# Jack-Tattershall/mujoco-manip

Measured on AMD Instinct MI355X. Metric: env steps/sec (whole node) at 4096 parallel envs; 1/2/4/8 MI355X scaling, higher is better.
Workload: dtype f32

## Files before the change

mujoco_manip_amd/_build.py:

```python
from __future__ import annotations

import os
import subprocess
from concurrent.futures import ThreadPoolExecutor

PKG = os.path.dirname(os.path.abspath(__file__))
CSRC = os.path.join(PKG, "csrc")
LIB = os.path.join(PKG, "libmmx.so")
LIB_PROF = os.path.join(PKG, "libmmx_prof.so")
SOURCES = ["mmx_kernels.hip", "mmx_step_l192.hip", "mmx_render.hip", "mmx_render_lit.hip", "mmx_png.hip",
           "mmx_snapshot.hip", "mmx_mppi.hip", "mmx_policy.hip", "mmx_api.cpp"]
ARCH = os.environ.get("MMX_OFFLOAD_ARCH", "gfx950")
DEVICE_MATH = ["-Xarch_device", "-freciprocal-math", "-Xarch_device", "-fapprox-func",
               "-Xarch_device", "-ffinite-math-only", "-Xarch_device", "-fno-signed-zeros"]
DEVICE_SCHED = ["-mllvm", "-amdgpu-sched-strategy=" + os.environ.get("MMX_SCHED", "iterative-ilp")]
if os.environ.get("MMX_SCHED") == "default":
    DEVICE_SCHED = []
DEVICE_NOSLP = ["-Xarch_device", "-fno-slp-vectorize"]
FLAGS = DEVICE_MATH + DEVICE_SCHED + DEVICE_NOSLP + os.environ.get("MMX_EXTRA_FLAGS", "").split()
SOURCE_FLAGS = {"mmx_kernels.hip": ["-Xarch_device", "-fassociative-math"],
                "mmx_step_l192.hip": ["-Xarch_device", "-fassociative-math"],
                "mmx_mppi.hip": ["-Xarch_device", "-fno-finite-math-only"]}


STEP_SOURCES = ["mmx_kernels.hip", "mmx_step_l192.hip"]
HIPCC_JOBS = 16
TEST_VARIANTS = {
    "libmmx_col4.so": ["MMX_COL_LIST=4", "MMX_CAND_CAP=4"],
    "libmmx_nolist.so": ["MMX_CAND_CAP=1"],
    "libmmx_hdelay.so": ["MMX_HELPER_DELAY=1", "MMX_PROBE=14"],
    "libmmx_edelay.so": ["MMX_HELPER_DELAY=2", "MMX_PROBE=14"],
    "libmmx_synth.so": ["MMX_BUDGET_SYNTH=1"],
}


def lib_path(profile: bool = False) -> str:
    return LIB_PROF if profile else LIB


def test_variant(name: str) -> str:
    path = os.path.join(PKG, name)
    if not os.path.exists(path):
        raise RuntimeError("test build missing: run __graft_entry__.build()")
    return path


def _stale(lib: str) -> bool:
    if not os.path.exists(lib):
        return True
    t = os.path.getmtime(lib)
    inc = os.path.join(PKG, "..", "include")
    deps = [os.path.join(CSRC, f) for f in os.listdir(CSRC) if f.endswith((".hip", ".cpp", ".h", ".inc"))]
    deps += [os.path.join(inc, f) for f in os.listdir(inc) if f.endswith(".h")]
    return any(os.path.getmtime(d) > t for d in deps)


def _hipcc(src: str, obj: str, defines: list[str] | tuple = (), profile: bool = False, verbose: bool = False) -> str:
    cmd = [os.environ.get("HIPCC", "/opt/rocm/bin/hipcc")] + (["-xhip"] if src.endswith(".cpp") else [])
    cmd += FLAGS + SOURCE_FLAGS.get(src, []) + [f"-D{d}" for d in defines] + (["-DMMX_PHASE_CLOCK=1"] if profile else [])
    cmd += [f"--offload-arch={ARCH}", "-O3", "-std=c++17", "-fPIC", "-c", os.path.join(CSRC, src), "-o", obj]
    if verbose:
        print(" ".join(cmd), flush=True)
    subprocess.check_call(cmd)
    return obj


def _link(out: str, objs: list[str]) -> str:
    subprocess.check_call([os.environ.get("HIPCC", "/opt/rocm/bin/hipcc"), f"--offload-arch={ARCH}", "-shared", "-fPIC", "-o", out] + objs)
    return out


def _obj(src: str, tag: str = "") -> str:
    return os.path.join(CSRC, os.path.splitext(src)[0] + tag + ".o")


def build(force: bool = False, verbose: bool = False, profile: bool | None = False) -> str:
    variants = [False, True] if profile is None else [profile]
    variants = [v for v in variants if force or _stale(lib_path(v))]
    tests = [n for n in TEST_VARIANTS if profile is None and (force or _stale(os.path.join(PKG, n)))]
    if variants or tests:
        pdef = [f"MMX_PROBE={int(os.environ.get('MMX_PROBE', '1'))}"]
        jobs = [(src, v) for v in variants for src in SOURCES]
        tjobs = [(n, src) for n in tests for src in STEP_SOURCES]
        with ThreadPoolExecutor(max_workers=min(HIPCC_JOBS, len(jobs) + len(tjobs))) as ex:
            tobjs = [ex.submit(_hipcc, src, _obj(src, "_" + os.path.splitext(n)[0]), TEST_VARIANTS[n], False, verbose)
                     for n, src in tjobs]
            objs = list(ex.map(lambda j: _hipcc(j[0], _obj(j[0], "_prof" if j[1] else ""), pdef if j[1] else [], j[1], verbose), jobs))
            tobjs = [f.result() for f in tobjs]
        for v in variants:
            _link(lib_path(v), [o for o, (_, vv) in zip(objs, jobs) if vv == v])
        for n in tests:
            kobjs = [o for o, (nn, _) in zip(tobjs, tjobs) if nn == n]
            _link(os.path.join(PKG, n), kobjs + [_obj(src) for src in SOURCES if src not in STEP_SOURCES])
    return lib_path(bool(profile))


if __name__ == "__main__":
    print(build(force=True, verbose=True, profile=None))


def build_variant(out: str, defines: list[str], profile: bool = True) -> str:
    tag = os.path.splitext(os.path.basename(out))[0]
    where = os.path.dirname(os.path.abspath(out))
    os.makedirs(where, exist_ok=True)
    with ThreadPoolExecutor(max_workers=len(SOURCES)) as ex:
        objs = list(ex.map(lambda src: _hipcc(src, os.path.join(where, f"{tag}_{os.path.splitext(src)[0]}.o"), defines, profile), SOURCES))
    return _link(out, objs)
```

mujoco_manip_amd/csrc/mmx_geom.h:

```cpp
#ifndef MMX_GEOM_H
#define MMX_GEOM_H
#include "mmx_device.h"
#include "mmx_state.h"
#include "mmx_clock.h"

enum { GT_PLANE = 0, GT_CYL = 5, GT_BOX = 6, GT_MESH = 7 };

struct Geom {
  V3 x;
  M3 R;
  int type, g;
};

DEV V3 support(const Geom& G, V3 dir) {
  V3 dl = mulT(G.R, dir), sl;
  const int g = G.g;
  if (G.type == GT_BOX) {
    sl = V3{dl.x >= 0.f ? MMX_geom_size[3 * g] : -MMX_geom_size[3 * g],
            dl.y >= 0.f ? MMX_geom_size[3 * g + 1] : -MMX_geom_size[3 * g + 1],
            dl.z >= 0.f ? MMX_geom_size[3 * g + 2] : -MMX_geom_size[3 * g + 2]};
  } else if (G.type == GT_CYL) {
    const float r = MMX_geom_size[3 * g], hh = MMX_geom_size[3 * g + 1];
    const float n = sqrtf(dl.x * dl.x + dl.y * dl.y);
    sl = n > 1e-12f ? V3{r * dl.x / n, r * dl.y / n, 0.f} : V3{r, 0.f, 0.f};
    sl.z = dl.z >= 0.f ? hh : -hh;
  } else {
    const int m = MMX_geom_mesh[g];
    const int a = MMX_mesh_vertadr[m], nvert = MMX_mesh_vertnum[m];
    float best = -3.0e38f;
    int bi = a;
    for (int v = a; v < a + nvert; v++) {
      const float s = MMX_mesh_vert[3 * v] * dl.x + MMX_mesh_vert[3 * v + 1] * dl.y + MMX_mesh_vert[3 * v + 2] * dl.z;
      if (s > best) {
        best = s;
        bi = v;
      }
    }
    sl = V3{MMX_mesh_vert[3 * bi], MMX_mesh_vert[3 * bi + 1], MMX_mesh_vert[3 * bi + 2]};
  }
  return G.x + mul(G.R, sl);
}

DEV bool obb_overlap(const Geom& A, const Geom& B, V3 ha, V3 hb) {
  const V3 d = B.x - A.x;
  float Rm[3][3], aR[3][3];
#pragma unroll
  for (int i = 0; i < 3; i++)
#pragma unroll
    for (int j = 0; j < 3; j++) {
      Rm[i][j] = dot(col(A.R, i), col(B.R, j));
      aR[i][j] = fabsf(Rm[i][j]);
    }
  const float hA[3] = {ha.x, ha.y, ha.z}, hB[3] = {hb.x, hb.y, hb.z};
  bool sep = false;
#pragma unroll
  for (int i = 0; i < 3; i++) {
    const float t = dot(d, col(A.R, i));
    sep |= fabsf(t) > hA[i] + hB[0] * aR[i][0] + hB[1] * aR[i][1] + hB[2] * aR[i][2];
  }
#pragma unroll
  for (int j = 0; j < 3; j++) {
    const float u = dot(d, col(B.R, j));
    sep |= fabsf(u) > hB[j] + hA[0] * aR[0][j] + hA[1] * aR[1][j] + hA[2] * aR[2][j];
  }
  (void)Rm;
  return !sep;
}

template <class Sink>
DEV void plane_box(Sink& cs, const Geom& P, const Geom& B, V3 hb) {
  const V3 nz = col(P.R, 2);
  const float h[3] = {hb.x, hb.y, hb.z};
  float cd[8];
  V3 cp[8];
  int cnt = 0;
#pragma unroll
  for (int k = 0; k < 8; k++) {
    cd[k] = 0.f;
    cp[k] = V3{0.f, 0.f, 0.f};
  }
#pragma unroll
  for (int k = 0; k < 8; k++) {
    const V3 l = V3{(k & 1) ? h[0] : -h[0], (k & 2) ? h[1] : -h[1], (k & 4) ? h[2] : -h[2]};
    const V3 w = B.x + mul(B.R, l);
    const float d = dot(w - P.x, nz);
    if (d <= 0.f) {
      const V3 pw = w - nz * (0.5f * d);
// ... 359 lines not shown
  wave_argmax(best, bi);
  const int wl = bi & 63;
  const V3 p = V3{__int_as_float(__builtin_amdgcn_readlane(__float_as_int(bx), wl)),
                  __int_as_float(__builtin_amdgcn_readlane(__float_as_int(by), wl)),
                  __int_as_float(__builtin_amdgcn_readlane(__float_as_int(bz), wl))};
  return G.x + mul(G.R, p);
}

struct SVx {
  V3 w, a, b;
};
struct GPair {
  const Geom& A;
  const Geom& B;
};
DEV SVx mk_sv(const GPair& P, V3 dir) {
  SVx s;
  s.a = support_wave(P.A, dir);
  s.b = support_wave(P.B, -dir);
  s.w = s.a - s.b;
  return s;
}
DEV bool gjk_line(const SVx& s0, const SVx& s1, int& n, V3& dir) {
  const V3 ab = s1.w - s0.w, ao = -s0.w;
  if (dot(ab, ao) > 0.f) {
    dir = cross(cross(ab, ao), ab);
    n = 2;
    return norm(dir) < 1e-12f * (1.f + dot(ab, ab));
  }
  n = 1;
  dir = ao;
  return false;
}
DEV bool gjk_tri(const SVx& s0, SVx& s1, SVx& s2, int& n, V3& dir) {
  const V3 ab = s1.w - s0.w, ac = s2.w - s0.w, ao = -s0.w;
  const V3 abc = cross(ab, ac);
  if (dot(cross(abc, ac), ao) > 0.f) {
    if (dot(ac, ao) > 0.f) {
      s1 = s2;
      n = 2;
      dir = cross(cross(ac, ao), ac);
      return false;
    }
    n = 2;
    return gjk_line(s0, s1, n, dir);
  }
  if (dot(cross(ab, abc), ao) > 0.f) {
    n = 2;
    return gjk_line(s0, s1, n, dir);
  }
  const float dd = dot(abc, ao);
  n = 3;
  if (fabsf(dd) < 1e-12f * (1.f + dot(abc, abc))) return true;
  if (dd > 0.f) dir = abc;
  else {
    const SVx t = s1;
    s1 = s2;
    s2 = t;
    dir = -abc;
  }
  return false;
}
DEV bool gjk_face_out(const SVx& s0, const SVx& b, const SVx& c, const SVx& o) {
  V3 nn = cross(b.w - s0.w, c.w - s0.w);
  if (dot(nn, o.w - s0.w) > 0.f) nn = -nn;
  return dot(nn, -s0.w) > 0.f;
}
DEV bool gjk_tet(const SVx& s0, SVx& s1, SVx& s2, SVx& s3, int& n, V3& dir) {
  n = 3;
  if (gjk_face_out(s0, s1, s2, s3)) return gjk_tri(s0, s1, s2, n, dir);
  if (gjk_face_out(s0, s2, s3, s1)) {
    s1 = s2;
    s2 = s3;
    return gjk_tri(s0, s1, s2, n, dir);
  }
  if (gjk_face_out(s0, s3, s1, s2)) {
    s2 = s1;
    s1 = s3;
    return gjk_tri(s0, s1, s2, n, dir);
  }
  n = 4;
  return true;
}
DEV bool gjk(const GPair& GP, SVx& s0, SVx& s1, SVx& s2, SVx& s3, int& n) {
  V3 dir = GP.A.x - GP.B.x;
  if (norm(dir) < 1e-9f) dir = V3{1.f, 0.f, 0.f};
  s0 = mk_sv(GP, dir);
  n = 1;
  dir = -s0.w;
  for (int it = 0; it < 48; it++) {
    if (norm(dir) < 1e-12f) return true;
    const SVx P = mk_sv(GP, dir);
    if (dot(P.w, dir) < 0.f) return false;
    s3 = s2;
    s2 = s1;
    s1 = s0;
    s0 = P;
    n++;
    const bool hit = n == 2 ? gjk_line(s0, s1, n, dir)
                            : (n == 3 ? gjk_tri(s0, s1, s2, n, dir) : gjk_tet(s0, s1, s2, s3, n, dir));
    if (hit) return true;
  }
  return norm(dir) < 1e-12f;
}

#define EPA_MAXV 38
#define EPA_MAXF 72
struct EFace {
  int vv;
  V3 n;
  float d;
  DEV int v(int k) const { return (vv >> (8 * k)) & 255; }
};
static_assert(EPA_MAXV < 256, "EPA vertex indices are packed in bytes");
DEV bool epa_face(const SVx* V, EFace& f, int a, int b, int c) {
  f.vv = a | (b << 8) | (c << 16);
  const V3 n = cross(V[b].w - V[a].w, V[c].w - V[a].w);
  const float ln = norm(n);
  if (ln < 1e-20f) return false;
  f.n = n * (1.f / ln);
  f.d = dot(f.n, V[a].w);
  return true;
}
DEV void epa_sync() {
  __builtin_amdgcn_fence(__ATOMIC_RELEASE, "wavefront");
  __builtin_amdgcn_wave_barrier();
  __builtin_amdgcn_fence(__ATOMIC_ACQUIRE, "wavefront");
}
DEV int epa_lane() { return (int)(threadIdx.x & 63); }
DEV int epa_prefix(unsigned long long m) {
  return __builtin_amdgcn_mbcnt_hi((unsigned)(m >> 32), __builtin_amdgcn_mbcnt_lo((unsigned)m, 0u));
}
DEV bool epa(const GPair& GP, SVx* V, int nv, V3& nrm, float& depth, V3& pa, V3& pb, EFace* F, int* edges) {
  int nf = 0;
  if (nv == 1) {
    for (int k = 0; k < 6 && nv < 2; k++) {
      const float sg = (k & 1) ? -1.f : 1.f;
      V[nv] = mk_sv(GP, V3{k < 2 ? sg : 0.f, (k >> 1) == 1 ? sg : 0.f, k >= 4 ? sg : 0.f});
      if (norm(V[nv].w - V[0].w) > 1e-7f) nv++;
    }
  }
  if (nv == 2) {
    const V3 ab = V[1].w - V[0].w;
    const V3 ax = fabsf(ab.x) <= fabsf(ab.y) && fabsf(ab.x) <= fabsf(ab.z)
                      ? V3{1.f, 0.f, 0.f}
                      : (fabsf(ab.y) <= fabsf(ab.z) ? V3{0.f, 1.f, 0.f} : V3{0.f, 0.f, 1.f});
    const V3 t = normalize(cross(ab, ax));
    V[2] = mk_sv(GP, t);
    if (norm(cross(V[2].w - V[0].w, ab)) < 1e-10f) V[2] = mk_sv(GP, -t);
    nv = 3;
  }
  if (nv == 3) {
    const V3 n = normalize(cross(V[1].w - V[0].w, V[2].w - V[0].w));
    V[3] = mk_sv(GP, n);
    if (fabsf(dot(V[3].w - V[0].w, n)) < 1e-9f) V[3] = mk_sv(GP, -n);
    nv = 4;
  }
  const int T[4][3] = {{0, 1, 2}, {0, 3, 1}, {0, 2, 3}, {1, 3, 2}};
  const V3 cen = (V[0].w + V[1].w + V[2].w + V[3].w) * 0.25f;
  for (int k = 0; k < 4; k++) {
    if (!epa_face(V, F[nf], T[k][0], T[k][1], T[k][2])) continue;
    if (dot(F[nf].n, V[T[k][0]].w - cen) < 0.f) epa_face(V, F[nf], T[k][0], T[k][2], T[k][1]);
    nf++;
  }
  static_assert(EPA_MAXF <= 128, "two faces per lane");
  const int ln = epa_lane();
  int best = -1;
  for (;;) {
    epa_sync();
    float bd = -3e38f;
    int bi = 0x7fffffff;
    if (ln < nf && F[ln].d < 3e38f) {
      bd = -F[ln].d;
      bi = ln;
    }
// ... 3 lines not shown
    }
    wave_argmax(bd, bi);
    best = bi < nf ? bi : -1;
    if (best < 0) return false;
    const V3 fn = F[best].n;
    const float fd = F[best].d;
    const SVx P = mk_sv(GP, fn);
    const float dist = dot(P.w, fn);
    if (dist - fd < 1e-6f * (1.f + fabsf(dist)) || nv >= EPA_MAXV) break;
    EFace f0, f1;
    bool vis0 = false, vis1 = false;
    if (ln < nf) {
      f0 = F[ln];
      vis0 = dot(f0.n, P.w - V[f0.v(0)].w) > 1e-9f;
    }
    if (ln + 64 < nf) {
      f1 = F[ln + 64];
      vis1 = dot(f1.n, P.w - V[f1.v(0)].w) > 1e-9f;
    }
    const unsigned long long mv0 = __ballot(vis0), mv1 = __ballot(vis1);
    const unsigned long long mk0 = __ballot(ln < nf && !vis0), mk1 = __ballot(ln + 64 < nf && !vis1);
    int ne = 0;
    for (int half = 0; half < 2; half++) {
      unsigned long long m = half ? mv1 : mv0;
      while (m) {
        const int k = 64 * half + __builtin_ctzll(m);
        m &= m - 1ull;
        const EFace f = F[k];
        for (int e = 0; e < 3; e++) {
          const int a = f.v(e), b = f.v((e + 1) % 3);
          int found = -1;
          for (int q0 = 0; q0 < ne && found < 0; q0 += 64) {
            const int q = q0 + ln;
            const unsigned long long hit = __ballot(q < ne && edges[q] == (b | (a << 8)));
            if (hit) found = q0 + __builtin_ctzll(hit);
          }
          epa_sync();
          if (found >= 0) {
            if (ln == 0) edges[found] = edges[ne - 1];
            ne--;
          } else if (ne < EPA_MAXF * 3) {
            if (ln == 0) edges[ne] = a | (b << 8);
            ne++;
          }
          epa_sync();
        }
      }
    }
    epa_sync();
    const int nk0 = __popcll(mk0);
    if (ln < nf && !vis0) F[epa_prefix(mk0)] = f0;
    if (ln + 64 < nf && !vis1) F[nk0 + epa_prefix(mk1)] = f1;
    nf = nk0 + __popcll(mk1);
    const int pi = nv++;
    if (ln == 0) V[pi] = P;
    epa_sync();
    for (int q0 = 0; q0 < ne && nf < EPA_MAXF; q0 += 64) {
      const int q = q0 + ln;
      EFace g;
      const bool ok = q < ne && epa_face(V, g, edges[q] & 255, edges[q] >> 8, pi);
      const unsigned long long mo = __ballot(ok);
      const int pos = nf + epa_prefix(mo);
      if (ok && pos < EPA_MAXF) F[pos] = g;
      nf = min(EPA_MAXF, nf + __popcll(mo));
    }
  }
  epa_sync();
  if (best < 0) return false;
  const EFace& f = F[best];
  const V3 p = f.n * f.d;
  const V3 ra = V[f.v(0)].w - p, rb = V[f.v(1)].w - p, rc = V[f.v(2)].w - p;
  const float den = dot(cross(V[f.v(1)].w - V[f.v(0)].w, V[f.v(2)].w - V[f.v(0)].w), f.n);
  const float lu = den > 1e-15f ? dot(cross(rb, rc), f.n) / den : 1.f;
  const float lv = den > 1e-15f ? dot(cross(rc, ra), f.n) / den : 0.f;
  const float lw = 1.f - lu - lv;
  pa = V[f.v(0)].a * lu + V[f.v(1)].a * lv + V[f.v(2)].a * lw;
  pb = V[f.v(0)].b * lu + V[f.v(1)].b * lv + V[f.v(2)].b * lw;
  nrm = f.n;
  depth = f.d;
  return true;
}

#define EPA_SCRATCH_FLOATS (9 * EPA_MAXV + 5 * EPA_MAXF + 3 * EPA_MAXF)
template <class Sink>
DEV void convex_convex(Sink& cs, const Geom& A, const Geom& B, float* scr) {
  const GPair GP{A, B};
  SVx s0, s1, s2, s3;
  int n = 0;
  if (!gjk(GP, s0, s1, s2, s3, n)) return;
  SVx* V = reinterpret_cast<SVx*>(scr);
  EFace* F = reinterpret_cast<EFace*>(scr + 9 * EPA_MAXV);
  int* edges = reinterpret_cast<int*>(scr + 9 * EPA_MAXV + 5 * EPA_MAXF);
  V[0] = s0;
  if (n > 1) V[1] = s1;
  if (n > 2) V[2] = s2;
  if (n > 3) V[3] = s3;
  V3 nrm, pa, pb;
  float depth;
  if (!epa(GP, V, n, nrm, depth, pa, pb, F, edges)) return;
  if (depth < 0.f) return;
  if ((threadIdx.x & 63) == 0) cs.add(A.g, B.g, -depth, (pa + pb) * 0.5f, nrm);
}

DEV float impedance(const float* si, float pos) {
  const float dmin = fminf(fmaxf(si[0], 1e-4f), 0.9999f), dmax = fminf(fmaxf(si[1], 1e-4f), 0.9999f);
  const float width = si[2], mid = si[3], power = si[4];
  if (dmin == dmax || width <= 1e-15f) return 0.5f * (dmin + dmax);
  const float x = fabsf(pos / width);
  if (x >= 1.f) return dmax;
  if (x <= 0.f) return dmin;
  float y;
  if (power == 1.f) y = x;
  else if (power == 2.f) y = x <= mid ? x * x / mid : 1.f - (1.f - x) * (1.f - x) / (1.f - mid);
  else if (x <= mid) y = powf(x, power) / powf(mid, power - 1.f);
  else y = 1.f - powf(1.f - x, power) / powf(1.f - mid, power - 1.f);
  return dmin + y * (dmax - dmin);
}

#endif
```

mujoco_manip_amd/csrc/mmx_state.h:

```cpp
#ifndef MMX_STATE_H
#define MMX_STATE_H
#include <stdint.h>

#define MMX_NQ_ 30
#define MMX_NV_ 27
#define MMX_NU_ 8
#define MMX_NOBS 85
#define MMX_MAXCON 64
#define MMX_MAXEFC 320
#ifndef MMX_LDSEFC
#define MMX_LDSEFC 128
#endif
#define MMX_OVFEFC (MMX_MAXEFC - MMX_LDSEFC)
#ifndef MMX_CAND_CAP
#define MMX_CAND_CAP 256
#endif
#define MMX_OVF_ARROW_AT(efc) (18 * (MMX_MAXEFC - (efc)))
#define MMX_OVF_HDR_AT(efc) (MMX_OVF_ARROW_AT(efc) + 27 * 27 + 3)
#define MMX_OVF_CAND_AT(efc) (MMX_OVF_HDR_AT(efc) + (MMX_MAXEFC - (efc) + 3) / 4)
#define MMX_OVF_F_AT(efc) ((MMX_OVF_CAND_AT(efc) + (MMX_CAND_CAP + 1) / 2 + 3) / 4 * 4)
#define MMX_OVF_F MMX_OVF_F_AT(MMX_LDSEFC)
#define MMX_NSUBSTEP 16

enum {
  KIN_HAND_POS = 0,
  KIN_HAND_MAT = 3,
  KIN_AXIS = 12,
  KIN_ANCHOR = 33,
  KIN_OBJ = 54,
  KIN_N = 63
};

enum {
  EPI_OBJ = 0, EPI_BIN, EPI_STEP, EPI_FLAGS, EPI_FSM_STATE, EPI_FSM_TASKIDX, EPI_FSM_SETTLE,
  EPI_FSM_GRIP, EPI_FSM_HASTGT, EPI_ERROR, EPI_NCON, EPI_NEFC, EPI_EPISODES, EPI_RNG_HAS32,
  EPI_NSUCCESS, EPI_NPLACED, EPI_NERROR, EPI_PHASES,
  EPI_N
};
enum {
  EPF_TINIT = 0,
  EPF_HWM = 12,
  EPF_TGTKP = 17,
  EPF_FSM_TARGET = 21,
  EPF_FSM_TRANSIT = 24,
  EPF_EP_RETURN = 27,
  EPF_N = 28
};
enum { FLAG_GRASPED = 1, FLAG_LIFTED = 2, FLAG_ABOVE = 4, FLAG_PLACED = 8, FLAG_HWM_VALID = 16 };
enum { ERR_CON_OVERFLOW = 1, ERR_EFC_OVERFLOW = 2, ERR_NAN = 4, ERR_SAMPLING = 8 };

enum { CON_DIST = 0, CON_POS = 1, CON_N = 4, CON_MU0 = 7, CON_MU1, CON_MU2, CON_DIM, CON_G1, CON_G2, CON_F };
enum {
  STAT_NEFC = 0, STAT_NCON, STAT_SOLVER_ITER, STAT_SUBSTEPS, STAT_RESID,
  STAT_T_IK, STAT_T_KIN, STAT_T_DYN, STAT_T_COL, STAT_T_CON, STAT_T_SOLVE, STAT_T_INT, STAT_T_END,
  STAT_T_AUX0, STAT_T_AUX1, STAT_T_AUX2, STAT_T_AUX3,
  STAT_EXIT_STALL, STAT_EXIT_CAP,
  STAT_N
};

enum { MMX_SOLVER_NEWTON = 0, MMX_SOLVER_PGS = 1 };

struct MMXState {
  int N;
  int action_mode, reward_type, max_episode_steps, randomize, image_size, autoreset;
  double spawn_x0, spawn_x1, spawn_y0, spawn_y1;
  int ntask, task_obj[9], task_bin[9], fixed_obj, fixed_bin;
  int solver, solver_max_iter;
  float solver_tol;
  float* qpos;
  float* qvel;
  float* ctrl;
  float* qacc_ws;
  float* kin;
  float* target;
  int* epi;
  float* epf;
  unsigned long long* rng;
  unsigned int* rng32;
  float* obs;
  float* reward;
  float* reward_components;
  int* done;
  float* con;
  float* stats;
  float* efc_ovf;
  int* fault;
  float* rpose;
  unsigned char* images;
  unsigned char* seg;
  unsigned int* bg_overhead;
};

struct MMXTraj {
  float* obs;
  float* reward;
  int* done;
  float* reward_components;
  float* target;
  int* epi;
  float* qpos;
  float* qvel;
};

// ... 11 lines not shown
```

mujoco_manip_amd/csrc/mmx_step_collision.inc:

```
DEV Geom geom_pose(const EnvSh& E, int g) {
  Geom G;
  G.g = g;
  G.type = MMX_geom_type[g];
  const int b = MMX_geom_body[g];
  if (MMX_body_static[b]) {
    G.x = V3{MMX_geom_static_xpos[3 * g], MMX_geom_static_xpos[3 * g + 1], MMX_geom_static_xpos[3 * g + 2]};
#pragma unroll
    for (int k = 0; k < 9; k++) G.R.m[k] = MMX_geom_static_xmat[9 * g + k];
  } else {
    const V3 bx = body_x(E, b);
    const M3 bR = body_R(E, b);
    G.x = bx + mul(bR, V3{MMX_geom_pos[3 * g], MMX_geom_pos[3 * g + 1], MMX_geom_pos[3 * g + 2]});
    M3 Lm;
#pragma unroll
    for (int k = 0; k < 9; k++) Lm.m[k] = MMX_geom_lmat[9 * g + k];
    G.R = mul(bR, Lm);
  }
  return G;
}

struct WaveSink {
  EnvSh* E;
  int key;
  bool store;
// ... 167 lines not shown
  int ni = 0;
#pragma unroll
  for (int q = 0; q < NPASS; q++) {
    const unsigned long long m = km[q];
    if ((m >> LANE) & 1ull) {
      const int pos = __builtin_amdgcn_mbcnt_hi((unsigned)(m >> 32), __builtin_amdgcn_mbcnt_lo((unsigned)m, 0u));
      if (nc + pos < COL_LIST) cand[nc + pos] = cand_pack(q * WG + LANE, pg[q]);
    }
    nc += __popcll(m);
    if (rebuild) {
      const unsigned long long mi = ki[q];
      const int pos = __builtin_amdgcn_mbcnt_hi((unsigned)(mi >> 32), __builtin_amdgcn_mbcnt_lo((unsigned)mi, 0u));
      if (((mi >> LANE) & 1ull) && ni + pos < MMX_CAND_CAP) cand_of(E)[ni + pos] = (unsigned short)(q * WG + LANE);
      ni += __popcll(mi);
    }
  }
  if (rebuild) {
    __builtin_amdgcn_fence(__ATOMIC_SEQ_CST, "workgroup");
    if (LANE == 0) {
      E.ncand = ni <= MMX_CAND_CAP ? ni : -1;
      E.cdisp = 0.f;
    }
  }
  if (nc > COL_LIST) {
    if (LANE == 0) E.flags |= SHF_CON_OVF;
    nc = COL_LIST;
  }
  }
  SYNC();
  PROBE(2, stats, STAT_T_AUX1);
  constexpr int NCP = (COL_LIST + WG - 1) / WG;
  int ce[NCP];
  int ncls[3] = {0, 0, 0};
#pragma unroll
  for (int q = 0; q < NCP; q++) {
    const int k = q * WG + LANE;
    int c = 3, p = 0;
    if (q * WG < nc) {
      if (k < nc) {
        p = cand[k];
        int pp, g1, g2;
        cand_unpack(p, pp, g1, g2);
        const Geom A = geom_lds(gx, g1), B = geom_lds(gx, g2);
        if (A.type == GT_PLANE) c = 0;
        else if (obb_overlap(A, B, geom_half(gx, g1), geom_half(gx, g2))) c = (A.type == GT_BOX && B.type == GT_BOX) ? 1 : 2;
      }
#pragma unroll
      for (int t = 0; t < 3; t++) ncls[t] += __popcll(__ballot(c == t));
    }
    ce[q] = p | (c << 24);
  }
  SYNC();
  int base[3] = {0, ncls[0], ncls[0] + ncls[1]};
#pragma unroll
  for (int q = 0; q < NCP; q++) {
    if (q * WG < nc) {
      const int c = ce[q] >> 24;
#pragma unroll
      for (int t = 0; t < 3; t++) base[t] = wave_compact(c == t, cand, base[t], ce[q] & 0xFFFFFF);
    }
  }
  if (LANE == 0) {
    E.ncls[0] = ncls[0];
    E.ncls[1] = ncls[1];
    E.ncls[2] = ncls[2];
  }
  SYNC();
  if (MMX_PROBE == 4 && LANE == 0) {
    stats[STAT_T_AUX0] += (float)nc;
    stats[STAT_T_AUX1] += (float)ncls[1];
    stats[STAT_T_AUX2] += (float)ncls[2];
    stats[STAT_T_AUX3] += (float)ncls[0];
  }
  if (MMX_PROBE == 13 && LANE == 0 && !only_ro) {
    stats[STAT_T_AUX0] += use_list ? 0.f : 1.f;
    stats[STAT_T_AUX1] += (rebuild && E.ncand < 0) ? 1.f : 0.f;
    stats[STAT_T_AUX2] += (float)ncls[1];
    stats[STAT_T_AUX3] += (float)ncls[2];
  }
  if (MMX_PROBE == 14 && LANE == 0 && !only_ro) {
    stats[STAT_T_AUX0] += use_list ? 0.f : 1.f;
    stats[STAT_T_AUX1] = E.cdisp;
  }
  PROBE(2, stats, STAT_T_AUX2);
  PROBE(5, stats, STAT_T_AUX3);
}

DEV void collide_pairs(EnvSh& E, bool only_ro, int which) {
  float* stats = E.stats;
  CLK_DECL;
  float* scr = scr_of(E);
  const float* gx = scr + COL_GX;
  const int* cand = reinterpret_cast<const int*>(scr + COL_CAND);
  const int n0 = E.ncls[0], n1 = E.ncls[1], n2 = E.ncls[2];
  if (which & 1) {
    for (int k = LANE; k < n0; k += WG) {
      int p, g1, g2;
      cand_unpack(cand[k], p, g1, g2);
      const Geom A = geom_lds(gx, g1), B = geom_lds(gx, g2);
      WaveSink cs(&E, p, !only_ro, g1, g2);
      if (B.type == GT_BOX) plane_box(cs, A, B, geom_half(gx, g2));
      else if (B.type == GT_MESH) plane_convex(cs, A, B);
    }
    SYNC();
    PROBE(5, stats, STAT_T_AUX0);
    V3* poly = reinterpret_cast<V3*>(scr + COL_WORK + COL_POLY * (LANE >> 2));
    for (int k0 = 0; k0 < n1; k0 += WG / 4) {
      const int k = k0 + (LANE >> 2);
      if (k < n1) {
        int p, g1, g2;
        cand_unpack(cand[n0 + k], p, g1, g2);
        const Geom A = geom_lds(gx, g1), B = geom_lds(gx, g2);
        WaveSink cs(&E, p, !only_ro, g1, g2);
        box_box_quad(cs, A, B, geom_half(gx, g1), geom_half(gx, g2), poly, poly + 8);
      }
    }
    SYNC();
    PROBE(5, stats, STAT_T_AUX1);
  }
  if (which & 2) {
    for (int k = 0; k < n2; k++) {
      int p, g1, g2;
      cand_unpack(cand[n0 + n1 + k], p, g1, g2);
      const Geom A = geom_lds(gx, g1), B = geom_lds(gx, g2);
      WaveSink cs(&E, p, !only_ro, g1, g2);
      convex_convex(cs, A, B, scr + SCR_EPA);
    }
    SYNC();
    PROBE(5, stats, STAT_T_AUX2);
  }
}

DEV void collide_sort(EnvSh& E) {
  float* stats = E.stats;
  CLK_DECL;
  float* scr = scr_of(E);
  const int n = min(E.ncon, MMX_MAXCON);
  float* tmp = scr + COL_WORK;
  int kb = 0, rank = 0;
  if (LANE < n) {
    kb = con_key(crec(E, LANE));
    const int key = kb & 0xFFFF;
    for (int j = 0; j < n; j++) rank += (con_key(crec(E, j)) & 0xFFFF) < key;
#pragma unroll
    for (int f = 0; f < CL_F; f++) tmp[f * MMX_MAXCON + rank] = con_of(E)[f * MMX_MAXCON + LANE];
  }
  SYNC();
  for (int k = LANE; k < MMX_MAXCON * CL_F; k += WG) con_of(E)[k] = tmp[k];
  if (LANE == 0) E.ncon = n;
  SYNC();
  PROBE(5, stats, STAT_T_AUX3);
}

DEV void collide_wave(EnvSh& E, bool only_ro) {
  collide_prune(E, only_ro);
  collide_pairs(E, only_ro, 3);
  if (!only_ro) collide_sort(E);
}
```

mujoco_manip_amd/csrc/mmx_step_lds.inc:

```
enum { CL_DIST = 0, CL_POS = 1, CL_N = 4, CL_KEY = 7, CL_F };
static_assert(MMX_NGEOM <= 64 && MMX_NPAIR * 8 < 65536, "contact key packing");
struct CRec {
  const float* b;
  int c;
  DEV float operator[](int k) const { return b[k * MMX_MAXCON + c]; }
};
struct CRecW {
  float* b;
  int c;
  DEV float& operator[](int k) const { return b[k * MMX_MAXCON + c]; }
};
struct CReg {
  float v[CL_F];
  DEV float operator[](int k) const { return v[k]; }
};
template <class R>
DEV int con_key(const R& c) { return __float_as_int(c[CL_KEY]); }
template <class R>
DEV int con_g1(const R& c) { return (con_key(c) >> 16) & 63; }
template <class R>
DEV int con_g2(const R& c) { return (con_key(c) >> 22) & 63; }
#define GST 17
struct EnvSh {
  float qpos[30], qvel[28], ctrl[8];
// ... 20 lines not shown
  float cspd;
  int ncand;
};
static __shared__ EnvSh g_E;
static_assert(MMX_LDSEFC != 128 || (sizeof(EnvSh) + 1279) / 1280 * 1280 * 12 <= 160 * 1024,
              "EnvSh no longer fits 12 envs per CU");
static_assert((sizeof(EnvSh) + 1279) / 1280 * 1280 * 8 <= 160 * 1024, "EnvSh no longer fits 8 envs per CU");

#define GXS 17
#define GX_RB 12
#define GX_TYPE 13
#define GX_HALF 14
#define COL_GX 0
#define COL_CAND ((MMX_NGEOM * GXS + 15) & ~15)
#ifndef MMX_COL_LIST
#define MMX_COL_LIST 320
#endif
#define COL_LIST MMX_COL_LIST
#define COL_CON (COL_CAND + COL_LIST)
#define COL_WORK (COL_CON + CL_F * MMX_MAXCON)
#define COL_POLY 49
#define COL_PLANES 16
#define COL_EPA COL_WORK
static_assert(offsetof(EnvSh, hdr) == offsetof(EnvSh, J) + sizeof(EnvSh::J) &&
                  offsetof(EnvSh, D) == offsetof(EnvSh, hdr) + sizeof(EnvSh::hdr) &&
                  offsetof(EnvSh, NC) == offsetof(EnvSh, D) + sizeof(EnvSh::D) &&
                  offsetof(EnvSh, G) == offsetof(EnvSh, NC) + sizeof(EnvSh::NC),
              "the scratch region must be contiguous");
#define SCR_FLOATS ((int)((offsetof(EnvSh, G) + sizeof(EnvSh::G) - offsetof(EnvSh, J)) / 4))
static_assert(COL_EPA + EPA_SCRATCH_FLOATS <= SCR_FLOATS, "EPA scratch exceeds the scratch region");
static_assert(COL_WORK + MMX_MAXCON * CL_F <= SCR_FLOATS, "contact sort exceeds the scratch region");
static_assert(COL_CON % 4 == 0 && COL_WORK % 4 == 0, "16-byte aligned collision scratch blocks");
static_assert(COL_WORK + COL_PLANES * COL_POLY <= SCR_FLOATS, "box-box polygons exceed the scratch region");
static_assert(MMX_CAND_CAP <= COL_LIST && MMX_NPAIR < 4096, "collision scratch layout");

#ifndef MMX_STEP_HELPER
#define MMX_STEP_HELPER (MMX_LDSEFC == 192)
#endif
#if MMX_STEP_HELPER
#define COL_END (COL_WORK + EPA_SCRATCH_FLOATS)
static_assert(COL_WORK + COL_PLANES * COL_POLY <= COL_END && COL_WORK + MMX_MAXCON * CL_F <= COL_END,
              "the narrowphase work space exceeds COL_END");
#define SCR_DYN ((COL_END + 3) & ~3)
#define SCR_IKW SCR_DYN
#define SCR_EPA SCR_DYN
#else
#define SCR_DYN COL_WORK
#define SCR_IKW 0
#define SCR_EPA COL_EPA
#endif
#define SCR_IC (SCR_DYN + 272)
#define SCR_AF (SCR_IC + 120)
#define SCR_BIAS (SCR_AF + 8)
#define SCR_OBS COL_WORK
#define SCR_ACT (COL_WORK + 96)
static_assert(SCR_BIAS + 9 <= SCR_FLOATS && SCR_OBS + MMX_NOBS <= SCR_ACT && SCR_ACT + 12 <= SCR_FLOATS &&
                  SCR_EPA + EPA_SCRATCH_FLOATS <= SCR_FLOATS && SCR_IKW + 72 <= SCR_FLOATS,
              "scratch layout");
#ifndef MMX_HELPER_DELAY
#define MMX_HELPER_DELAY 0
#endif
#if MMX_HELPER_DELAY && MMX_STEP_HELPER
#define MMX_DELAY_SLEEPS 4
DEV void delay_wave() {
#pragma unroll
  for (int k = 0; k < MMX_DELAY_SLEEPS; k++) __builtin_amdgcn_s_sleep(127);
  asm volatile("" ::: "memory");
}
#define DELAY_HELPER() do { if (MMX_HELPER_DELAY == 1) delay_wave(); } while (0)
#define DELAY_ENV() do { if (MMX_HELPER_DELAY == 2) delay_wave(); } while (0)
#else
#define DELAY_HELPER() do { } while (0)
#define DELAY_ENV() do { } while (0)
#endif
DEV float* scr_of(EnvSh& E) { return reinterpret_cast<float*>(&E.J); }
DEV const float* scr_of(const EnvSh& E) { return reinterpret_cast<const float*>(&E.J); }
DEV float* obs_of(EnvSh& E) { return scr_of(E) + SCR_OBS; }
DEV const float* obs_of(const EnvSh& E) { return scr_of(E) + SCR_OBS; }
DEV float* con_of(EnvSh& E) { return scr_of(E) + COL_CON; }
DEV CRec crec(const EnvSh& E, int c) { return CRec{scr_of(E) + COL_CON, c}; }
DEV float* lrow_of(EnvSh& E) { return E.G; }
DEV float* arrow_of(EnvSh& E) { return E.ovf + MMX_OVF_ARROW_AT(MMX_LDSEFC); }
DEV unsigned short* cand_of(const EnvSh& E) { return reinterpret_cast<unsigned short*>(E.ovf + MMX_OVF_CAND_AT(MMX_LDSEFC)); }
static_assert(MMX_LDSEFC % WG == 0 && MMX_LDSEFC <= MMX_MAXEFC, "LDS rows: whole lane slices");
DEV float* ovf_j(const EnvSh& E, int i) { return E.ovf + 16 * (i - MMX_LDSEFC); }
DEV float* ovf_d(const EnvSh& E, int i) { return E.ovf + 16 * MMX_OVFEFC + (i - MMX_LDSEFC); }
DEV float* ovf_nc(const EnvSh& E, int i) { return E.ovf + 17 * MMX_OVFEFC + (i - MMX_LDSEFC); }
DEV float& jlds(EnvSh& E, int i, int k) { return E.J[k >> 2][i][k & 3]; }
DEV const float& jlds(const EnvSh& E, int i, int k) { return E.J[k >> 2][i][k & 3]; }
DEV float4 jrow4(const EnvSh& E, int i, int q) {
  if (i >= MMX_LDSEFC) return reinterpret_cast<const float4*>(ovf_j(E, i))[q];
  return *reinterpret_cast<const float4*>(E.J[q][i]);
}
DEV float jget(const EnvSh& E, int i, int k) { return i < MMX_LDSEFC ? jlds(E, i, k) : ovf_j(E, i)[k]; }
DEV void jset(EnvSh& E, int i, int k, float v) {
  if (i < MMX_LDSEFC) jlds(E, i, k) = v;
  else ovf_j(E, i)[k] = v;
}
DEV float dget(const EnvSh& E, int i) { return i < MMX_LDSEFC ? E.D[i] : *ovf_d(E, i); }
DEV void dset(EnvSh& E, int i, float v) {
  if (i < MMX_LDSEFC) E.D[i] = v;
  else *ovf_d(E, i) = v;
}
DEV float ncget(const EnvSh& E, int i) { return i < MMX_LDSEFC ? E.NC[i] : *ovf_nc(E, i); }
DEV unsigned char* ovf_hdr(const EnvSh& E) { return reinterpret_cast<unsigned char*>(E.ovf + MMX_OVF_HDR_AT(MMX_LDSEFC)); }
DEV int hdr_get(const EnvSh& E, int i) { return i < MMX_LDSEFC ? E.hdr[i] : ovf_hdr(E)[i - MMX_LDSEFC]; }
DEV void hdr_set(EnvSh& E, int i, int h) {
  if (i < MMX_LDSEFC) E.hdr[i] = (unsigned char)h;
  else ovf_hdr(E)[i - MMX_LDSEFC] = (unsigned char)h;
}
DEV void ncset(EnvSh& E, int i, float v) {
  if (i < MMX_LDSEFC) E.NC[i] = v;
  else *ovf_nc(E, i) = v;
}
DEV void ovf_fence(int nefc) {
  if (nefc > MMX_LDSEFC) __builtin_amdgcn_fence(__ATOMIC_SEQ_CST, "workgroup");
}
DEV void store_contacts(float* dst, const EnvSh& E) {
  const int n = E.ncon;
  for (int c = LANE; c < MMX_MAXCON; c += WG) {
    float* o = dst + (size_t)c * CON_F;
    const CRec l = crec(E, c);
    const int g1 = c < n ? con_g1(l) : 0, g2 = c < n ? con_g2(l) : 0;
    o[CON_DIST] = c < n ? l[CL_DIST] : 0.f;
#pragma unroll
    for (int k = 0; k < 3; k++) {
      o[CON_POS + k] = c < n ? l[CL_POS + k] : 0.f;
      o[CON_N + k] = c < n ? l[CL_N + k] : 0.f;
      o[CON_MU0 + k] = c < n ? fmaxf(MMX_geom_friction[3 * g1 + k], MMX_geom_friction[3 * g2 + k]) : 0.f;
    }
    o[CON_DIM] = c < n ? (float)max(MMX_geom_condim[g1], MMX_geom_condim[g2]) : 0.f;
    o[CON_G1] = c < n ? (float)g1 : 0.f;
    o[CON_G2] = c < n ? (float)g2 : 0.f;
  }
}
DEV float* contacts_dst(const MMXState& S, int i) { return S.con + (size_t)i * MMX_MAXCON * CON_F; }
enum { SHF_ROBOT_OBST = 1, SHF_CON_OVF = 2, SHF_EFC_OVF = 4, SHF_NAN = 8 };

DEV int body_slot(int b) { return b <= 11 ? b - 1 : b - 5; }
DEV float& kin_ref(EnvSh& E, int k) {
  if (k < KIN_HAND_MAT) return E.bx[body_slot(MMX_BODY_HAND)][k - KIN_HAND_POS];
  if (k < KIN_AXIS) return E.bR[body_slot(MMX_BODY_HAND)][k - KIN_HAND_MAT];
  if (k < KIN_ANCHOR) return E.S[(k - KIN_AXIS) / 3][(k - KIN_AXIS) % 3];
  if (k < KIN_OBJ) return E.bx[body_slot(MMX_jnt_body[(k - KIN_ANCHOR) / 3])][(k - KIN_ANCHOR) % 3];
  return E.bx[11 + (k - KIN_OBJ) / 3][(k - KIN_OBJ) % 3];
}
DEV float kin_get(const EnvSh& E, int k) { return kin_ref(const_cast<EnvSh&>(E), k); }
DEV int body_block(int b) { return (b >= 2 && b <= 11) ? 0 : (b >= 16 ? b - 15 : -1); }
#define BLK_NONE 15
DEV int blk_size(int b) { return b == 0 ? 9 : (b == BLK_NONE ? 0 : 6); }
DEV int blk_d0(int b) { return b == 0 ? 0 : 9 + 6 * (b - 1); }
DEV int dof_blk(int a) { return a < 9 ? 0 : 1 + (a - 9) / 6; }
DEV int row_slot(int h, int a) {
  const int b0 = h & 15, b1 = (h >> 4) & 15, ba = dof_blk(a);
  if (ba == b0) return a - blk_d0(b0);
  if (ba == b1) return blk_size(b0) + a - blk_d0(b1);
  return -1;
}
#define NTYPE 10
static constexpr int kTB0[NTYPE] = {0, 0, 0, 0, 1, 1, 1, 2, 2, 3};
static constexpr int kTB1[NTYPE] = {15, 1, 2, 3, 15, 2, 3, 15, 3, 15};
DEV int row_type(int b0, int b1) {
  return b0 == 0 ? (b1 == BLK_NONE ? 0 : b1) : (b0 == 1 ? (b1 == BLK_NONE ? 4 : 3 + b1) : (b0 == 2 ? (b1 == BLK_NONE ? 7 : 8) : 9));
}
DEV bool arm_anc(int d, int b) { return d <= 6 ? (b >= d + 2 && b <= 11) : (d == 7 ? b == 10 : b == 11); }
DEV unsigned anc_mask(int b) {
// ... 58 lines not shown
```

Measured before the change: 3.406 million.

## Cache GJK separating axes per env pair to skip full GJK on repeat

```diff
diff --git a/mujoco_manip_amd/_build.py b/mujoco_manip_amd/_build.py
--- a/mujoco_manip_amd/_build.py
+++ b/mujoco_manip_amd/_build.py
@@ -28,6 +28,8 @@
 TEST_VARIANTS = {
     "libmmx_col4.so": ["MMX_COL_LIST=4", "MMX_CAND_CAP=4"],
     "libmmx_nolist.so": ["MMX_CAND_CAP=1"],
+    "libmmx_nocache.so": ["MMX_GJK_CACHE=0", "MMX_PROBE=15"],
+    "libmmx_gjkprobe.so": ["MMX_PROBE=15"],
     "libmmx_hdelay.so": ["MMX_HELPER_DELAY=1", "MMX_PROBE=14"],
     "libmmx_edelay.so": ["MMX_HELPER_DELAY=2", "MMX_PROBE=14"],
     "libmmx_synth.so": ["MMX_BUDGET_SYNTH=1"],
diff --git a/mujoco_manip_amd/csrc/mmx_geom.h b/mujoco_manip_amd/csrc/mmx_geom.h
--- a/mujoco_manip_amd/csrc/mmx_geom.h
+++ b/mujoco_manip_amd/csrc/mmx_geom.h
@@ -3,6 +3,7 @@
 #include "mmx_device.h"
 #include "mmx_state.h"
 #include "mmx_clock.h"
+#include "mmx_gjk_cache.h"
 
 enum { GT_PLANE = 0, GT_CYL = 5, GT_BOX = 6, GT_MESH = 7 };
 
@@ -528,15 +529,17 @@
   n = 4;
   return true;
 }
-DEV bool gjk(const GPair& GP, SVx& s0, SVx& s1, SVx& s2, SVx& s3, int& n) {
-  V3 dir = GP.A.x - GP.B.x;
+DEV bool gjk(const GPair& GP, SVx& s0, SVx& s1, SVx& s2, SVx& s3, int& n, V3& dir, int& rounds) {
+  dir = GP.A.x - GP.B.x;
   if (norm(dir) < 1e-9f) dir = V3{1.f, 0.f, 0.f};
   s0 = mk_sv(GP, dir);
+  rounds = 1;
   n = 1;
   dir = -s0.w;
   for (int it = 0; it < 48; it++) {
     if (norm(dir) < 1e-12f) return true;
     const SVx P = mk_sv(GP, dir);
+    rounds++;
     if (dot(P.w, dir) < 0.f) return false;
     s3 = s2;
     s2 = s1;
@@ -706,12 +709,87 @@
 }
 
 #define EPA_SCRATCH_FLOATS (9 * EPA_MAXV + 5 * EPA_MAXF + 3 * EPA_MAXF)
+struct AxisCache {
+  float* tab = nullptr;
+  int tag = 0;
+  float x = 0.f, y = 0.f, z = 0.f;
+  unsigned busy = 0u;
+};
+DEV void axis_cache_load(AxisCache& ac, float* tab) {
+  ac.tab = tab;
+  if ((int)(threadIdx.x & 63) < MMX_AXIS_SLOTS) {
+    const float4 e = *reinterpret_cast<const float4*>(tab + MMX_AXIS_WORDS * (int)(threadIdx.x & 63));
+    ac.tag = __float_as_int(e.x);
+    ac.x = e.y;
+    ac.y = e.z;
+    ac.z = e.w;
+  }
+}
+#define GJK_PROBE15(st, k, v)                                                          \
+  do {                                                                                 \
+    if (MMX_PROBE == 15 && (threadIdx.x & 63) == 0) (st)[k] += (float)(v);             \
+  } while (0)
 template <class Sink>
-DEV void convex_convex(Sink& cs, const Geom& A, const Geom& B, float* scr) {
+DEV void convex_convex(Sink& cs, const Geom& A, const Geom& B, float* scr, AxisCache& ac, int pair) {
   const GPair GP{A, B};
+  float* st = cs.E->stats;
+  const int lane = (int)(threadIdx.x & 63);
+  GJK_PROBE15(st, STAT_T_AUX0, 1);
+  unsigned hit = 0u;
+#if MMX_GJK_CACHE
+  if (ac.tab) {
+    hit = (unsigned)__ballot(lane < MMX_AXIS_SLOTS && ac.tag == pair + 1);
+    if (hit) {
+      const int h = __ffs((int)hit) - 1;
+      const int tag = __builtin_amdgcn_readlane(ac.tag, h);
+      const V3 d = V3{__int_as_float(__builtin_amdgcn_readlane(__float_as_int(ac.x), h)),
+                      __int_as_float(__builtin_amdgcn_readlane(__float_as_int(ac.y), h)),
+                      __int_as_float(__builtin_amdgcn_readlane(__float_as_int(ac.z), h))};
+      ac.busy |= 1u << h;
+      if (gjkc_dir_ok(d.x, d.y, d.z)) {
+        const SVx P = mk_sv(GP, d);
+        GJK_PROBE15(st, STAT_T_AUX2, 1);
+        if (gjkc_separated(tag, pair, d.x, d.y, d.z, P.w.x, P.w.y, P.w.z)) {
+          GJK_PROBE15(st, STAT_T_AUX1, 1);
+          GJK_PROBE15(st, STAT_T_AUX3, 1);
+          return;
+        }
+      }
+    }
+  }
+#endif
   SVx s0, s1, s2, s3;
-  int n = 0;
-  if (!gjk(GP, s0, s1, s2, s3, n)) return;
+  int n = 0, rounds = 0;
+  V3 dir;
+  const bool pen = gjk(GP, s0, s1, s2, s3, n, dir, rounds);
+  GJK_PROBE15(st, STAT_T_AUX2, rounds);
+  GJK_PROBE15(st, STAT_T_AUX1, pen ? 0 : 1);
+#if MMX_GJK_CACHE
+  if (ac.tab) {
+    if (!pen) {
+      const int s = gjkc_slot(hit, ac.busy, pair);
+      V3 dn = dir * (1.f / norm(dir));
+      asm volatile("" : "+v"(dn.x), "+v"(dn.y), "+v"(dn.z));
+      if (s >= 0 && gjkc_dir_ok(dn.x, dn.y, dn.z)) {
+        ac.busy |= 1u << s;
+        if (lane == s) {
+          ac.tag = pair + 1;
+          ac.x = dn.x;
+          ac.y = dn.y;
+          ac.z = dn.z;
+          *reinterpret_cast<float4*>(ac.tab + MMX_AXIS_WORDS * s) = make_float4(__int_as_float(pair + 1), dn.x, dn.y, dn.z);
+        }
+      }
+    } else if (hit) {
+      const int h = __ffs((int)hit) - 1;
+      if (lane == h) {
+        ac.tag = 0;
+        ac.tab[MMX_AXIS_WORDS * h] = 0.f;
+      }
+    }
+  }
+#endif
+  if (!pen) return;
   SVx* V = reinterpret_cast<SVx*>(scr);
   EFace* F = reinterpret_cast<EFace*>(scr + 9 * EPA_MAXV);
   int* edges = reinterpret_cast<int*>(scr + 9 * EPA_MAXV + 5 * EPA_MAXF);
diff --git a/mujoco_manip_amd/csrc/mmx_gjk_cache.h b/mujoco_manip_amd/csrc/mmx_gjk_cache.h
--- /dev/null
+++ b/mujoco_manip_amd/csrc/mmx_gjk_cache.h
@@ -0,0 +1,60 @@
+#ifndef MMX_GJK_CACHE_H
+#define MMX_GJK_CACHE_H
+#include <stdint.h>
+#include <string.h>
+
+#if defined(__HIPCC__)
+#include <hip/hip_runtime.h>
+#define GJKC_HD __host__ __device__ inline
+#else
+#define GJKC_HD inline
+#endif
+#if defined(__HIP_DEVICE_COMPILE__)
+#define GJKC_OPAQUE(v) asm volatile("" : "+v"(v))
+#else
+#define GJKC_OPAQUE(v) (void)0
+#endif
+
+#ifndef MMX_GJK_CACHE
+#define MMX_GJK_CACHE 1
+#endif
+#define MMX_AXIS_SLOTS 8
+#define MMX_AXIS_WORDS 4
+static_assert(MMX_AXIS_SLOTS <= 32, "the slot masks are 32-bit");
+
+#define MMX_AXIS_MARGIN 1e-5f
+
+GJKC_HD uint32_t gjkc_bits(float v) {
+  uint32_t b;
+  memcpy(&b, &v, 4);
+  return b;
+}
+GJKC_HD bool gjkc_component_ok(float v) { return (gjkc_bits(v) & 0x7fffffffu) <= 0x3f810000u; }
+GJKC_HD bool gjkc_dir_ok(float x, float y, float z) {
+  return gjkc_component_ok(x) && gjkc_component_ok(y) && gjkc_component_ok(z);
+}
+GJKC_HD bool gjkc_separated(int tag, int pair, float dx, float dy, float dz, float wx, float wy, float wz) {
+  if (tag != pair + 1 || !gjkc_dir_ok(dx, dy, dz)) return false;
+  const float n2 = dx * dx + dy * dy + dz * dz;
+  float s = wx * dx + wy * dy + wz * dz;
+  GJKC_OPAQUE(s);
+  const bool finite = (gjkc_bits(s) & 0x7f800000u) != 0x7f800000u;
+  return finite && n2 <= 1.001f && s < -MMX_AXIS_MARGIN;
+}
+GJKC_HD int gjkc_slot(unsigned hit, unsigned busy, int pair) {
+  const unsigned all = (1u << MMX_AXIS_SLOTS) - 1u;
+  hit &= all;
+  if (hit) {
+    int s = 0;
+    while (!((hit >> s) & 1u)) s++;
+    return s;
+  }
+  const int s0 = (int)((unsigned)pair % MMX_AXIS_SLOTS);
+  for (int k = 0; k < MMX_AXIS_SLOTS; k++) {
+    const int s = (s0 + k) % MMX_AXIS_SLOTS;
+    if (!((busy >> s) & 1u)) return s;
+  }
+  return -1;
+}
+
+#endif
diff --git a/mujoco_manip_amd/csrc/mmx_state.h b/mujoco_manip_amd/csrc/mmx_state.h
--- a/mujoco_manip_amd/csrc/mmx_state.h
+++ b/mujoco_manip_amd/csrc/mmx_state.h
@@ -1,6 +1,8 @@
 #ifndef MMX_STATE_H
 #define MMX_STATE_H
 #include <stdint.h>
+
+#include "mmx_gjk_cache.h"
 
 #define MMX_NQ_ 30
 #define MMX_NV_ 27
@@ -18,7 +20,8 @@
 #define MMX_OVF_ARROW_AT(efc) (18 * (MMX_MAXEFC - (efc)))
 #define MMX_OVF_HDR_AT(efc) (MMX_OVF_ARROW_AT(efc) + 27 * 27 + 3)
 #define MMX_OVF_CAND_AT(efc) (MMX_OVF_HDR_AT(efc) + (MMX_MAXEFC - (efc) + 3) / 4)
-#define MMX_OVF_F_AT(efc) ((MMX_OVF_CAND_AT(efc) + (MMX_CAND_CAP + 1) / 2 + 3) / 4 * 4)
+#define MMX_OVF_AXIS_AT(efc) ((MMX_OVF_CAND_AT(efc) + (MMX_CAND_CAP + 1) / 2 + 3) / 4 * 4)
+#define MMX_OVF_F_AT(efc) (MMX_OVF_AXIS_AT(efc) + MMX_AXIS_SLOTS * MMX_AXIS_WORDS)
 #define MMX_OVF_F MMX_OVF_F_AT(MMX_LDSEFC)
 #define MMX_NSUBSTEP 16
 
diff --git a/mujoco_manip_amd/csrc/mmx_step_collision.inc b/mujoco_manip_amd/csrc/mmx_step_collision.inc
--- a/mujoco_manip_amd/csrc/mmx_step_collision.inc
+++ b/mujoco_manip_amd/csrc/mmx_step_collision.inc
@@ -273,6 +273,12 @@
     stats[STAT_T_AUX0] += use_list ? 0.f : 1.f;
     stats[STAT_T_AUX1] = E.cdisp;
   }
+  if (MMX_PROBE == 16 && LANE == 0 && !only_ro) {
+    stats[STAT_T_AUX0] = fmaxf(stats[STAT_T_AUX0], (float)ncls[2]);
+    stats[STAT_T_AUX1] += ncls[2] > 2 ? 1.f : 0.f;
+    stats[STAT_T_AUX2] += ncls[2] > 4 ? 1.f : 0.f;
+    stats[STAT_T_AUX3] += ncls[2] > MMX_AXIS_SLOTS ? 1.f : 0.f;
+  }
   PROBE(2, stats, STAT_T_AUX2);
   PROBE(5, stats, STAT_T_AUX3);
 }
@@ -284,6 +290,8 @@
   const float* gx = scr + COL_GX;
   const int* cand = reinterpret_cast<const int*>(scr + COL_CAND);
   const int n0 = E.ncls[0], n1 = E.ncls[1], n2 = E.ncls[2];
+  AxisCache ac;
+  if (MMX_GJK_CACHE && (which & 2) && !only_ro && n2 > 0) axis_cache_load(ac, axis_of(E));
   if (which & 1) {
     for (int k = LANE; k < n0; k += WG) {
       int p, g1, g2;
@@ -315,7 +323,7 @@
       cand_unpack(cand[n0 + n1 + k], p, g1, g2);
       const Geom A = geom_lds(gx, g1), B = geom_lds(gx, g2);
       WaveSink cs(&E, p, !only_ro, g1, g2);
-      convex_convex(cs, A, B, scr + SCR_EPA);
+      convex_convex(cs, A, B, scr + SCR_EPA, ac, p);
     }
     SYNC();
     PROBE(5, stats, STAT_T_AUX2);
diff --git a/mujoco_manip_amd/csrc/mmx_step_lds.inc b/mujoco_manip_amd/csrc/mmx_step_lds.inc
--- a/mujoco_manip_amd/csrc/mmx_step_lds.inc
+++ b/mujoco_manip_amd/csrc/mmx_step_lds.inc
@@ -126,6 +126,7 @@
 DEV float* lrow_of(EnvSh& E) { return E.G; }
 DEV float* arrow_of(EnvSh& E) { return E.ovf + MMX_OVF_ARROW_AT(MMX_LDSEFC); }
 DEV unsigned short* cand_of(const EnvSh& E) { return reinterpret_cast<unsigned short*>(E.ovf + MMX_OVF_CAND_AT(MMX_LDSEFC)); }
+DEV float* axis_of(const EnvSh& E) { return E.ovf + MMX_OVF_AXIS_AT(MMX_LDSEFC); }
 static_assert(MMX_LDSEFC % WG == 0 && MMX_LDSEFC <= MMX_MAXEFC, "LDS rows: whole lane slices");
 DEV float* ovf_j(const EnvSh& E, int i) { return E.ovf + 16 * (i - MMX_LDSEFC); }
 DEV float* ovf_d(const EnvSh& E, int i) { return E.ovf + 16 * MMX_OVFEFC + (i - MMX_LDSEFC); }
```

Measured after the change: 3.473 million (median of 6 runs). +2.0%, better.
